# ywyue/AGILE3D

Measured on AMD Instinct MI355X. Metric: scenes/s (80k-voxel, 10 clicks), higher is better.
Workload: dtype f32; 1 GPU; batch of 16 synthetic 79736-voxel scenes, 10 clicks each (5 objects x 2), scene build + forward_backbone + 1 forward_mask per scene, fp32, eval; voxels=79736, queries=20, parallelism=scene-sharded x1 (no data-path collective), global_batch=16, steps_in_flight_per_gpu=4

## Files before the change

### agile3d_amd/csrc/decoder.hip

```cpp
#include "common.h"
#include <algorithm>
#include <type_traits>
#include <vector>

namespace a3d {

typedef float f32x4 __attribute__((ext_vector_type(4)));
#define A3D_GLOBAL __attribute__((address_space(1)))
template <typename T>
__device__ __forceinline__ T gld(const T* p) { return *(const T A3D_GLOBAL*)p; }
template <typename T>
__device__ __forceinline__ void gst(T* p, T v) { *(T A3D_GLOBAL*)p = v; }
__device__ __forceinline__ f32x4 gld4(const float* p) { return *(const f32x4 A3D_GLOBAL*)p; }
__device__ __forceinline__ void gst4(float* p, f32x4 v) { *(f32x4 A3D_GLOBAL*)p = v; }
__device__ __forceinline__ bool block_any(int pred, int* slot) {
  if (threadIdx.x == 0) *slot = 0;
  __syncthreads();
  if (pred) *slot = 1;
  __syncthreads();
  return *(volatile int*)slot != 0;
}
template <typename T>
__device__ __forceinline__ T gld_agent(const T* p) {
  return __hip_atomic_load((const T A3D_GLOBAL*)p, __ATOMIC_RELAXED, __HIP_MEMORY_SCOPE_AGENT);
// ... 17 lines not shown
  return fmaxf(__uint_as_float(b[0]), __uint_as_float(b[1]));
}
__device__ __forceinline__ float rows_sum(float x) {
  auto a = __builtin_amdgcn_permlane16_swap(__float_as_uint(x), __float_as_uint(x), false, false);
  x = __uint_as_float(a[0]) + __uint_as_float(a[1]);
  auto b = __builtin_amdgcn_permlane32_swap(__float_as_uint(x), __float_as_uint(x), false, false);
  return __uint_as_float(b[0]) + __uint_as_float(b[1]);
}
__device__ __forceinline__ float fast_exp(float x) { return __builtin_amdgcn_exp2f(x * 1.4426950408889634f); }
constexpr float kLog2e = 1.4426950408889634f;
constexpr float kPointScoreScale = 0.25f * kLog2e;
__device__ __forceinline__ float exp2_fast(float x) { return __builtin_amdgcn_exp2f(x); }

__device__ __forceinline__ f32x4 mfma4(float a, float b, f32x4 c) { return __builtin_amdgcn_mfma_f32_4x4x1f32(a, b, c, 0, 0, 0); }
__device__ __forceinline__ float rows_sum_scatter(f32x4 s) {
  auto a = __builtin_amdgcn_permlane32_swap(__float_as_uint(s[0]), __float_as_uint(s[1]), false, false);
  auto b = __builtin_amdgcn_permlane32_swap(__float_as_uint(s[2]), __float_as_uint(s[3]), false, false);
  const float r01 = __uint_as_float(a[0]) + __uint_as_float(a[1]);
  const float r23 = __uint_as_float(b[0]) + __uint_as_float(b[1]);
  auto c = __builtin_amdgcn_permlane16_swap(__float_as_uint(r01), __float_as_uint(r23), false, false);
  return __uint_as_float(c[0]) + __uint_as_float(c[1]);
}
__device__ __forceinline__ int row_reg(int g) { return ((g & 1) << 1) | (g >> 1); }
__device__ __forceinline__ float row_bcast(float x, int lane4, int row) {
  return __int_as_float(__builtin_amdgcn_ds_bpermute(lane4 + 64 * row, __float_as_int(x)));
}
__device__ __forceinline__ float quads_max(float x) {
  x = fmaxf(x, __shfl_xor(x, 4, 64));
  return fmaxf(x, __shfl_xor(x, 8, 64));
}
__device__ __forceinline__ float quads_sum(float x) {
  x += __shfl_xor(x, 4, 64);
  return x + __shfl_xor(x, 8, 64);
}

constexpr int kPosBlocks = 16;
struct PosBatch {
  int ns;
  int start[64 + 1];
};
__global__ void __launch_bounds__(256) k_minmax_partial_b(const float* __restrict__ xyz, const PosBatch pb, float* part) {
  __shared__ float s[6][256];
  const int b = blockIdx.y, r0 = pb.start[b], r1 = pb.start[b + 1];
  float mn[3] = {3.4e38f, 3.4e38f, 3.4e38f}, mx[3] = {-3.4e38f, -3.4e38f, -3.4e38f};
  for (int i = r0 + blockIdx.x * 256 + threadIdx.x; i < r1; i += gridDim.x * 256) {
#pragma unroll
    for (int a = 0; a < 3; ++a) {
      const float v = xyz[3 * (size_t)i + a];
      mn[a] = fminf(mn[a], v);
      mx[a] = fmaxf(mx[a], v);
    }
  }
#pragma unroll
  for (int a = 0; a < 3; ++a) {
    s[a][threadIdx.x] = mn[a];
    s[3 + a][threadIdx.x] = mx[a];
  }
  __syncthreads();
  for (int o = 128; o > 0; o >>= 1) {
    if (threadIdx.x < o) {
#pragma unroll
      for (int a = 0; a < 3; ++a) {
        s[a][threadIdx.x] = fminf(s[a][threadIdx.x], s[a][threadIdx.x + o]);
        s[3 + a][threadIdx.x] = fmaxf(s[3 + a][threadIdx.x], s[3 + a][threadIdx.x + o]);
      }
    }
    __syncthreads();
  }
  if (threadIdx.x < 6) part[((size_t)b * gridDim.x + blockIdx.x) * 6 + threadIdx.x] = s[threadIdx.x][0];
}
__global__ void k_minmax_final(const float* __restrict__ part, int nb, float* minmax) {
  part += (size_t)blockIdx.x * nb * 6;
  minmax += 6 * blockIdx.x;
  const int a = threadIdx.x >> 6, lane = threadIdx.x & 63;
  float v = a < 3 ? 3.4e38f : -3.4e38f;
  for (int b = lane; b < nb; b += 64) v = a < 3 ? fminf(v, part[b * 6 + a]) : fmaxf(v, part[b * 6 + a]);
#pragma unroll
  for (int o = 32; o > 0; o >>= 1) {
    const float w = __shfl_xor(v, o, 64);
    v = a < 3 ? fminf(v, w) : fmaxf(v, w);
  }
  if (lane == 0) minmax[a] = v;
}
template <bool NORM>
__device__ __forceinline__ void fourier_row(const float* __restrict__ xyz, size_t i, int jj, const float* __restrict__ gaussB,
                                            const float* __restrict__ minmax, float* out) {
  const float two_pi = 6.283185307179586f;
  float p = 0.f;
#pragma unroll
  for (int a = 0; a < 3; ++a) {
    float u = xyz[3 * i + a];
    if (NORM) {
      const float mn = minmax[a], mx = minmax[3 + a];
      u = (u - mn) / (mx - mn);
    }
    u *= two_pi;
    p += u * gaussB[a * 64 + jj];
  }
  float sn, cs;
  sincosf(p, &sn, &cs);
  out[i * D + jj] = sn;
  out[i * D + 64 + jj] = cs;
}
template <bool NORM>
__global__ void k_fourier_b(const float* __restrict__ xyz, const PosBatch pb, const float* __restrict__ gaussB,
                            const float* __restrict__ minmax, float* out) {
  const int b = blockIdx.y, r0 = pb.start[b], r1 = pb.start[b + 1];
  const size_t e = (size_t)blockIdx.x * blockDim.x + threadIdx.x;
  const size_t i = (size_t)r0 + (e >> 6);
  if (i >= (size_t)r1) return;
  fourier_row<NORM>(xyz, i, (int)(e & 63), gaussB, minmax + 6 * b, out);
}

__device__ const float kSineDimT[64] = {
    1.0f, 1.519911f, 2.3101296f, 3.5111918f, 5.3366995f, 8.111309f, 12.328468f, 18.738173f,
    28.480362f, 43.287613f, 65.79333f, 100.0f, 151.99113f, 231.01291f, 351.11914f, 533.6699f,
    811.131f, 1232.8464f, 1873.8174f, 2848.0361f, 4328.762f, 6579.331f, 1.0f, 1.5505158f,
    2.4040992f, 3.727594f, 5.779693f, 8.961505f, 13.894957f, 21.54435f, 33.404854f, 51.79475f,
    80.30857f, 124.51974f, 193.06982f, 299.3578f, 464.15897f, 719.6858f, 1115.8842f, 1730.1959f,
    2682.696f, 4159.5625f, 6449.467f, 1.0f, 1.5505158f, 2.4040992f, 3.727594f, 5.779693f,
    8.961505f, 13.894957f, 21.54435f, 33.404854f, 51.79475f, 80.30857f, 124.51974f, 193.06982f,
    299.3578f, 464.15897f, 719.6858f, 1115.8842f, 1730.1959f, 2682.696f, 4159.5625f, 6449.467f};
template <bool NORM>
__device__ __forceinline__ void sine_quad(const float* __restrict__ xyz, size_t i, int c4, const float* __restrict__ minmax,
                                          float* out) {
  const float two_pi = 6.283185307179586f;
  float4 v;
  float* vp = &v.x;
#pragma unroll
  for (int h = 0; h < 2; ++h) {
    const int p = 2 * c4 + h;
    const int a = (p >= 22) + (p >= 43);
    float u = xyz[3 * i + a];
    if (NORM) {
      const float mn = minmax[a], mx = minmax[3 + a];
      u = (u - mn) / (mx - mn);
    }
    u *= two_pi;
    sincosf(u / kSineDimT[p], &vp[2 * h], &vp[2 * h + 1]);
  }
  *reinterpret_cast<float4*>(out + i * D + 4 * c4) = v;
}
template <bool NORM>
__global__ void k_sine_b(const float* __restrict__ xyz, const PosBatch pb, const float* __restrict__ minmax, float* out) {
  const int b = blockIdx.y, r0 = pb.start[b], r1 = pb.start[b + 1];
  const size_t e = (size_t)blockIdx.x * blockDim.x + threadIdx.x;
  const size_t i = (size_t)r0 + (e >> 5);
  if (i >= (size_t)r1) return;
  sine_quad<NORM>(xyz, i, (int)(e & 31), minmax + 6 * b, out);
}

constexpr int kLegRows = 32, kLegF = 22, kLegLd = 6 * kLegF;
__device__ __forceinline__ void legacy_rows(const float* __restrict__ xyz, size_t r0, int rows, const float* __restrict__ inv_freq,
                                            float* out, float (*s)[kLegLd]) {
  for (int t = threadIdx.x; t < rows * 3 * kLegF; t += blockDim.x) {
    const int r = t / (3 * kLegF), q = t - 3 * kLegF * r, a = q / kLegF, j = q - kLegF * a;
    float sn, cs;
    sincosf(xyz[3 * (r0 + r) + a] * inv_freq[j], &sn, &cs);
    s[r][2 * kLegF * a + j] = sn;
    s[r][2 * kLegF * a + kLegF + j] = cs;
  }
  __syncthreads();
  for (int t = threadIdx.x; t < rows * 32; t += blockDim.x) {
    const int r = t >> 5, c4 = t & 31;
    *reinterpret_cast<float4*>(out + (r0 + r) * D + 4 * c4) = *reinterpret_cast<const float4*>(&s[r][4 * c4]);
  }
}
__global__ void __launch_bounds__(256) k_legacy_b(const float* __restrict__ xyz, const PosBatch pb,
                                                  const float* __restrict__ inv_freq, float* out) {
  __shared__ __align__(16) float s[kLegRows][kLegLd];
  const int b = blockIdx.y, r1 = pb.start[b + 1];
  const size_t r0 = (size_t)pb.start[b] + (size_t)blockIdx.x * kLegRows;
  if (r0 >= (size_t)r1) return;
  legacy_rows(xyz, r0, (int)((size_t)r1 - r0 < (size_t)kLegRows ? (size_t)r1 - r0 : (size_t)kLegRows), inv_freq, out, s);
}

struct QueryMeta {
  int n_fg, n_bg_click, n_bgl, nq, K;
  int row[A3D_MAX_QUERIES];
  int time[A3D_MAX_QUERIES];
  int obj[A3D_MAX_QUERIES];
  int qrange[A3D_MAX_QUERIES + 2];
};

struct QueryBufs {
  float *queries, *qpos, *qproj, *ks, *vs, *E;
  float *attn, *tmp, *tgt, *qk, *vc, *hidden;
  unsigned* sync;
};
constexpr int kQlMaxHelpers = 8;
constexpr int kMaxQBlocks = A3D_MAX_QUERIES / 32;

struct QuerySample {
  const QueryMeta* meta;
// ... 1989 lines not shown
        for (int t = 0; t < 4; ++t) facc[qt][t] += gld_agent(part + (size_t)(qt * 16 + 4 * g + t) * D + 16 * wave + j);
    }
  }
  qstore_b<QT>(facc, vec_l[V_FFN_B2 + cw], 1.f, false, xa, kQLD, 16 * wave, QP);
  __syncthreads();
  qln16<QT>(cur, xa, Q, vec_l + V_FFN_NW, vec_l + V_FFN_NB, cur, deleg ? nullptr : xa, qpos, B.queries, deleg ? B.tgt : nullptr);
  if (deleg) {
    __builtin_amdgcn_s_waitcnt(0x0F70);
    __syncthreads();
    if (tid == 0) gst_agent(flags + 8, 1u);
  } else {
    __syncthreads();
  }
  qln16<QT>(cur, nullptr, Q, vec_l + V_DN_W, vec_l + V_DN_B, xb, nullptr, nullptr, nullptr, nullptr);
  if (!deleg) {
    qzero<QT>(acc);
    qmm<QT>(xa, wfd, acc);
    qstore_b<QT, true>(acc, vec_l[V_S2C_IN_B + D + cw], kPointScoreScale, false, B.ks, D, 16 * wave, Q);
    qload_p(W.mpack + kMpW0, 8, wave, 0, wfd);
    qzero<QT>(acc);
    qmm<QT>(cur, wfa, acc);
    qstore_b<QT, true>(acc, vec_l[V_S2C_IN_B + 2 * D + cw], 1.f, false, B.vs, D, 16 * wave, Q);
    qload_p(W.mpack + kMpW2, 8, wave, 0, wfa);
    if (W.next_c2s_in_wt) {
      qload_p(W.next_qpack + kQpC2sQ, 8, wave, 0, wfb);
      qzero<QT>(acc);
      qmm<QT>(xa, wfb, acc);
      qstore_b<QT, true>(acc, vec_l[V_NEXT_B + cw], kPointScoreScale, false, B.qproj, D, 16 * wave, Q);
    }
  }
  __syncthreads();
  qzero<QT>(acc);
  qmm<QT>(xb, wfd, acc);
  qstore_b<QT>(acc, vec_l[V_M_B0 + cw], 1.f, true, qpos, kQLD, 16 * wave, QP);
  __syncthreads();
  qzero<QT>(acc);
  qmm<QT>(qpos, wfa, acc);
  qstore_b<QT, true>(acc, vec_l[V_M_B2 + cw], 1.f, false, B.E, D, 16 * wave, Q);
}

}

using namespace a3d;

static int posenc_run(const char* who, int kind, int normalize, const float* xyz_dev, const int64_t* starts, int n_samples,
                      int part_blocks, const float* table_dev, float* minmax_dev, float* out_dev, void* workspace_dev,
                      size_t workspace_bytes, void* stream) {
  if (kind != A3D_POSENC_FOURIER && kind != A3D_POSENC_SINE && kind != A3D_POSENC_LEGACY) {
    set_error("%s: unknown encoding kind %d", who, kind);
    return A3D_ERR_INVALID;
  }
  const bool mm = normalize && kind != A3D_POSENC_LEGACY;
  if ((kind != A3D_POSENC_SINE && !table_dev) || (mm && !minmax_dev) || !out_dev) {
    set_error("%s: bad arguments (table_dev: gauss_B / inv_freq; minmax_dev where the encoding normalises)", who);
    return A3D_ERR_INVALID;
  }
  if (!xyz_dev || !starts || n_samples < 1 || n_samples > 64) {
    set_error("%s: bad arguments (1..64 samples)", who);
    return A3D_ERR_INVALID;
  }
  PosBatch pb;
  pb.ns = n_samples;
  int n_max = 0;
  for (int b = 0; b <= n_samples; ++b) {
    if (starts[b] < 0 || starts[b] > ((int64_t)1 << 30) || (b && starts[b] <= starts[b - 1])) {
      set_error("%s: sample %d has no rows (1..2^30 rows in all, starts must ascend)", who, b - 1);
      return A3D_ERR_INVALID;
    }
    pb.start[b] = (int)starts[b];
    if (b) n_max = std::max(n_max, pb.start[b] - pb.start[b - 1]);
  }
  const size_t part_bytes = (size_t)n_samples * part_blocks * 6 * 4;
  if (mm && (!workspace_dev || workspace_bytes < part_bytes)) {
    set_error("%s: workspace needs >= %zu bytes", who, part_bytes);
    return A3D_ERR_WORKSPACE;
  }
  hipStream_t st = (hipStream_t)stream;
  ProfScope ps(st, A3D_PROF_POSENC, 0, 0, 3, 128, pb.start[n_samples]);
  if (mm) {
    k_minmax_partial_b<<<dim3(part_blocks, n_samples), 256, 0, st>>>(xyz_dev, pb, (float*)workspace_dev);
    k_minmax_final<<<n_samples, 384, 0, st>>>((const float*)workspace_dev, part_blocks, minmax_dev);
  }
  if (kind == A3D_POSENC_FOURIER) {
    const dim3 g((unsigned)(((size_t)n_max * 64 + 255) / 256), n_samples);
    if (mm) k_fourier_b<true><<<g, 256, 0, st>>>(xyz_dev, pb, table_dev, minmax_dev, out_dev);
    else k_fourier_b<false><<<g, 256, 0, st>>>(xyz_dev, pb, table_dev, nullptr, out_dev);
  } else if (kind == A3D_POSENC_SINE) {
    const dim3 g((unsigned)(((size_t)n_max * 32 + 255) / 256), n_samples);
    if (mm) k_sine_b<true><<<g, 256, 0, st>>>(xyz_dev, pb, minmax_dev, out_dev);
    else k_sine_b<false><<<g, 256, 0, st>>>(xyz_dev, pb, nullptr, out_dev);
  } else {
    k_legacy_b<<<dim3((unsigned)((n_max + kLegRows - 1) / kLegRows), n_samples), 256, 0, st>>>(xyz_dev, pb, table_dev, out_dev);
  }
  A3D_LAUNCH_CHECK();
  return A3D_OK;
}
static int posenc_one(const char* who, int kind, int normalize, const float* xyz_dev, int64_t n, const float* table_dev,
                      float* minmax_dev, float* out_dev, void* workspace_dev, size_t workspace_bytes, void* stream) {
  if (n <= 0 || n > (int64_t)1 << 30) {
    set_error("%s: bad arguments", who);
    return A3D_ERR_INVALID;
  }
  const int64_t starts[2] = {0, n};
  const int nb = (int)((n + 255) / 256 < 256 ? (n + 255) / 256 : 256);
  return posenc_run(who, kind, normalize, xyz_dev, starts, 1, nb, table_dev, minmax_dev, out_dev, workspace_dev,
                    workspace_bytes, stream);
}

extern "C" size_t a3d_posenc_batch_workspace_bytes(int n_samples) {
  return n_samples >= 1 && n_samples <= 64 ? (size_t)n_samples * kPosBlocks * 6 * 4 : 0;
}
static int posenc_aligned(const char* who, const float* out_dev) {
  if (((uintptr_t)out_dev & 15) == 0) return A3D_OK;
  set_error("%s: out_dev must be 16-byte aligned", who);
  return A3D_ERR_INVALID;
}
extern "C" int a3d_posenc(int kind, int normalize, const float* xyz_dev, int64_t n, const float* table_dev, float* minmax_dev,
                          float* out_dev, void* workspace_dev, size_t workspace_bytes, void* stream) {
  if (int rc = posenc_aligned("a3d_posenc", out_dev)) return rc;
  return posenc_one("a3d_posenc", kind, normalize, xyz_dev, n, table_dev, minmax_dev, out_dev, workspace_dev,
                    workspace_bytes, stream);
}
extern "C" int a3d_posenc_batch(int kind, int normalize, const float* xyz_dev, const int64_t* starts_host, int n_samples,
                                const float* table_dev, float* minmax_dev, float* out_dev, void* workspace_dev,
                                size_t workspace_bytes, void* stream) {
  if (int rc = posenc_aligned("a3d_posenc_batch", out_dev)) return rc;
  return posenc_run("a3d_posenc_batch", kind, normalize, xyz_dev, starts_host, n_samples, kPosBlocks, table_dev,
                    minmax_dev, out_dev, workspace_dev, workspace_bytes, stream);
}
extern "C" int a3d_posenc_fourier(const float* xyz_dev, int64_t n, const float* gauss_B_dev, float* minmax_dev,
                                  float* out_dev, void* workspace_dev, size_t workspace_bytes, void* stream) {
  return posenc_one("a3d_posenc_fourier", A3D_POSENC_FOURIER, 1, xyz_dev, n, gauss_B_dev, minmax_dev, out_dev,
                    workspace_dev, workspace_bytes, stream);
}
extern "C" int a3d_posenc_fourier_batch(const float* xyz_dev, const int64_t* starts_host, int n_samples,
                                        const float* gauss_B_dev, float* minmax_dev, float* out_dev, void* workspace_dev,
                                        size_t workspace_bytes, void* stream) {
  return posenc_run("a3d_posenc_fourier_batch", A3D_POSENC_FOURIER, 1, xyz_dev, starts_host, n_samples, kPosBlocks,
                    gauss_B_dev, minmax_dev, out_dev, workspace_dev, workspace_bytes, stream);
}

static int check_weights(const a3d_decoder_weights* w) {
  if (!w || w->n_layers < 1 || w->n_layers > A3D_MAX_DEC_LAYERS || w->n_bg_queries < 0 ||
      w->n_bg_queries > A3D_MAX_QUERIES || w->dim_ff % 128 != 0) {
    set_error("decoder: bad weight struct");
    return A3D_ERR_INVALID;
  }
  return A3D_OK;
}

static int check_packs(const a3d_decoder_weights* w) {
  if (!w->mask_pack) {
    set_error("a3d_decoder_forward: the decoder weights carry no mask-head pack (a3d_decoder_pack_query_weights fills "
              "a3d_decoder_layer::query_pack and a3d_decoder_weights::mask_pack)");
    return A3D_ERR_INVALID;
  }
  for (int l = 0; l < w->n_layers; ++l)
    if (!w->layers[l].query_pack) {
      set_error("a3d_decoder_forward: decoder layer %d carries no query-side pack (a3d_decoder_pack_query_weights fills "
                "a3d_decoder_layer::query_pack and a3d_decoder_weights::mask_pack)", l);
      return A3D_ERR_INVALID;
    }
  return A3D_OK;
}

namespace {
struct DecLayout {
  size_t buf[4], labels, counts, part, meta, desc, q[12], sync, total;
  int qp, nchunk;
// ... 749 lines not shown
```

### agile3d_amd/csrc/spconv.hip

```cpp
#include "common.h"
#include <algorithm>

namespace a3d {

typedef float f32x4 __attribute__((ext_vector_type(4)));

struct ConvArgs {
  const float* in;
  int ldi, n_in;
  const int* nbr;
  int nbr_stride;
  const uint32_t* gmask;
  const float* w;
  int K, cin, cout;
  float* out;
  int ldo, n_out;
  const int* out_map;
  const float* scale;
  const float* shift;
  const float* res;
  int ldr;
  int relu;
  int zero_row;
  int tag_table, tag_level;
// ... 1100 lines not shown
    }
  }
  __syncthreads();
  while (grp < ngroups) {
    f32x4 a[NS];
#pragma unroll
    for (int S = 0; S < NS; ++S) {
      if constexpr (HAS2) a[S] = nx[S] + nx2[S];
      else a[S] = nx[S];
    }
    const int next = grp + stride;
    if (next < ngroups) fetch(next);
    f32x4 acc[NCT];
#pragma unroll
    for (int ct = 0; ct < NCT; ++ct) acc[ct] = (f32x4){0.f, 0.f, 0.f, 0.f};
    {
      static_assert(NCT % 2 == 0, "pairs of 16-column tiles");
      constexpr int NP = NS * NCT / 2;
      const f32x4* Ws = Wl + lane;
      f32x4 c0 = Ws[0], c1 = Ws[64];
#pragma unroll
      for (int pi = 0; pi < NP; ++pi) {
        const int S = pi / (NCT / 2), ct = 2 * (pi % (NCT / 2));
        f32x4 n0 = c0, n1 = c1;
        if (pi + 1 < NP) {
          n0 = Ws[(2 * pi + 2) * 64];
          n1 = Ws[(2 * pi + 3) * 64];
        }
        __builtin_amdgcn_sched_barrier(0);
#pragma unroll
        for (int t = 0; t < 4; ++t) {
          acc[ct] = __builtin_amdgcn_mfma_f32_16x16x4f32(c0[t], a[S][t], acc[ct], 0, 0, 0);
          acc[ct + 1] = __builtin_amdgcn_mfma_f32_16x16x4f32(c1[t], a[S][t], acc[ct + 1], 0, 0, 0);
        }
        __builtin_amdgcn_sched_barrier(0);
        c0 = n0;
        c1 = n1;
      }
    }
    if (grp * 16 + j < n) {
      const int row = out_map ? out_map[grp * 16 + j] : grp * 16 + j;
#pragma unroll
      for (int ct = 0; ct < NCT; ++ct) {
        const int col = 16 * ct + 4 * g;
        f32x4 v = acc[ct];
        if (scale) v *= *(const f32x4*)(scale + col);
        if (shift) v += *(const f32x4*)(shift + col);
        if (res) v += *(const f32x4*)(res + (size_t)row * ldr + col);
        if (relu) {
#pragma unroll
          for (int t = 0; t < 4; ++t) v[t] = fmaxf(v[t], 0.f);
        }
        *(f32x4*)(Y + (size_t)row * ldy + col) = v;
      }
    }
    grp = next;
  }
}

static bool dense_supported(int cin, int cout) {
  return (cin == 96 || cin == 128) && (cout == 96 || cout == 128);
}
static int launch_dense(const float* X, int ldx, const float* X2, int ldx2, int n, int cin, int cout, const float* Wp,
                        const float* scale, const float* shift, const float* res, int ldr, int relu, float* Y,
                        int ldy, int zero_row, int tag_level, const int* out_map, hipStream_t st) {
  if ((ldx | ldx2 | ldr | ldy) & 3) {
    set_error("a3d_linear: leading dimensions must be multiples of 4");
    return A3D_ERR_INVALID;
  }
  const int ngroups = (n + 15) / 16;
  const int nw = n >= 200000 ? 12 : 4, wg_per_cu = n >= 200000 ? 1 : 2;
  const size_t lds = (size_t)(cin / 16) * (cout / 16) * 1024;
  ProfScope ps(st, A3D_PROF_DENSE, 0, 1, cin, cout, n, A3D_OP_LINEAR, tag_level, 1);
  const int max_grid = 256 * wg_per_cu;
  const int grid = (ngroups + nw - 1) / nw < max_grid ? (ngroups + nw - 1) / nw : max_grid;
#define A3D_DENSE(NS_, NCT_) (X2 ? big_lds<k_dense<NS_, NCT_, true>>() : big_lds<k_dense<NS_, NCT_, false>>())
  const auto kern = cin == 128 ? (cout == 128 ? A3D_DENSE(8, 8) : A3D_DENSE(8, 6)) : (cout == 128 ? A3D_DENSE(6, 8) : A3D_DENSE(6, 6));
#undef A3D_DENSE
  kern<<<grid, 64 * nw, lds, st>>>(X, ldx, X2, ldx2, n, Wp, scale, shift, res, ldr, relu, Y, ldy, ngroups, zero_row, out_map);
  A3D_LAUNCH_CHECK();
  return A3D_OK;
}

template <int NT, int KS>
__global__ void __launch_bounds__(NT) k_stem(const int32_t* __restrict__ xyzb, int n,
                                              const uint64_t* __restrict__ hk, const int* __restrict__ hv,
                                              uint32_t hmask, const f32x4* __restrict__ feats4,
                                              const float* __restrict__ w, int ,
                                              const float* __restrict__ scale, const float* __restrict__ shift,
                                              int relu, float* out, int ldo, int zero_row, const Level glv) {
  extern __shared__ __attribute__((aligned(16))) char smem[];
  constexpr int ks = KS, K = KS * KS * KS;
  float* W = (float*)smem;
  int* nb = (int*)(W + K * 96);
  const int tid = threadIdx.x;
  for (int e = tid; e < K * 96; e += NT) W[e] = w[e];
  const int v0 = blockIdx.x * 64;
  const int h = ks / 2;
  constexpr int TPV = NT / 64, CPT = 32 / TPV;
  constexpr int SEG = (K + TPV - 1) / TPV;
  const int v = tid / TPV, cg = tid % TPV;
  const bool fused = glv.grid && n < (1 << 25);
  const int mrow = v0 + v;
  const int row = fused ? (mrow < n ? glv.perm[mrow] : n) : mrow;
  int mine[SEG];
  if (fused) {
    int4 c = (int4){0, 0, 0, 0};
    if (mrow < n) {
      int b_, X_, Y_, Z_;
      decode_key(glv.keys[mrow], 0, b_, X_, Y_, Z_);
      c = (int4){X_, Y_, Z_, b_};
    }
#pragma unroll
    for (int u = 0; u < SEG; ++u) {
      const int k = cg * SEG + u;
      mine[u] = -1;
      if (k < K && row < n)
        mine[u] = glv.grid[grid_cell(glv, c.w, c.x + (k % ks) - h, c.y + ((k / ks) % ks) - h, c.z + (k / (ks * ks)) - h)];
    }
  } else if (glv.grid) {
    for (int e0 = tid; e0 < 64 * K; e0 += 8 * NT) {
      int res[8];
#pragma unroll
      for (int u = 0; u < 8; ++u) {
        const int e = e0 + u * NT;
        const int vv = e / K, k = e - vv * K;
        const int rr = v0 + vv;
        res[u] = -1;
        if (e < 64 * K && rr < n) {
          const int4 c = *(const int4*)(xyzb + 4 * rr);
          res[u] = glv.grid[grid_cell(glv, c.w, c.x + (k % ks) - h, c.y + ((k / ks) % ks) - h, c.z + (k / (ks * ks)) - h)];
          if (res[u] >= 0) res[u] = glv.perm[res[u]];
        }
      }
#pragma unroll
      for (int u = 0; u < 8; ++u)
        if (e0 + u * NT < 64 * K) nb[e0 + u * NT] = res[u];
    }
  } else
  for (int e0 = tid; e0 < 64 * K; e0 += 4 * NT) {
    uint64_t key[4];
    uint32_t hh[4];
    int res[4];
    bool open[4];
#pragma unroll
    for (int u = 0; u < 4; ++u) {
      const int e = e0 + u * NT;
      const int v = e / K, k = e - v * K;
      const int row = v0 + v;
      res[u] = -1;
      open[u] = false;
      key[u] = 0;
      hh[u] = 0;
      if (e < 64 * K && row < n) {
        const int X = xyzb[4 * row + 0] + (k % ks) - h;
        const int Y = xyzb[4 * row + 1] + ((k / ks) % ks) - h;
        const int Z = xyzb[4 * row + 2] + (k / (ks * ks)) - h;
        const int b = xyzb[4 * row + 3];
        const int lim = kCoordOff;
        if (X >= -lim && X < lim && Y >= -lim && Y < lim && Z >= -lim && Z < lim) {
          key[u] = make_key(b, X, Y, Z, 0);
          hh[u] = hash64(key[u]) & hmask;
          open[u] = true;
        }
      }
    }
    for (uint32_t probe = 0; probe <= hmask; ++probe) {
      uint64_t got[4];
#pragma unroll
      for (int u = 0; u < 4; ++u) got[u] = open[u] ? hk[hh[u]] : kEmptyKey;
      bool any = false;
#pragma unroll
      for (int u = 0; u < 4; ++u) {
        if (!open[u]) continue;
        if (got[u] == key[u]) {
          res[u] = hv[hh[u]];
          open[u] = false;
        } else if (got[u] == kEmptyKey) {
          open[u] = false;
        } else {
          hh[u] = (hh[u] + 1) & hmask;
          any = true;
        }
      }
      if (!any) break;
    }
#pragma unroll
    for (int u = 0; u < 4; ++u)
      if (e0 + u * NT < 64 * K) nb[e0 + u * NT] = res[u];
  }
  __syncthreads();
  float acc[CPT];
#pragma unroll
  for (int c = 0; c < CPT; ++c) acc[c] = 0.f;
  if (n < (1 << 25)) {
    constexpr int seg = SEG;
    int cnt = 0;
#pragma unroll
    for (int u = 0; u < SEG; ++u) {
      const int k = cg * seg + u;
      if (!fused) mine[u] = k < K ? nb[v * K + k] : -1;
      cnt += mine[u] >= 0 ? 1 : 0;
    }
    int incl = cnt;
#pragma unroll
    for (int o = 1; o < TPV; o <<= 1) {
      const int t = __shfl_up(incl, o, 64);
      if (cg >= o) incl += t;
    }
    const int total = __shfl(incl, (threadIdx.x & 63) | (TPV - 1), 64);
    if (!fused) __syncthreads();
    int pos = incl - cnt;
#pragma unroll
    for (int u = 0; u < SEG; ++u)
      if (mine[u] >= 0) nb[v * K + pos++] = (int)((uint32_t)mine[u] | ((uint32_t)(cg * seg + u) << 25));
    __syncthreads();
    for (int i0 = 0; i0 < total; i0 += 8) {
      uint32_t e[8];
      f32x4 f[8];
#pragma unroll
      for (int u = 0; u < 8; ++u) e[u] = i0 + u < total ? (uint32_t)nb[v * K + i0 + u] : 0u;
#pragma unroll
      for (int u = 0; u < 8; ++u) f[u] = feats4[e[u] & 0x1ffffffu];
#pragma unroll
      for (int u = 0; u < 8; ++u) {
        if (i0 + u >= total) continue;
        const float* wk = W + (e[u] >> 25) * 96 + cg * CPT;
#pragma unroll
        for (int c = 0; c < CPT; ++c) acc[c] += f[u][0] * wk[c] + f[u][1] * wk[32 + c] + f[u][2] * wk[64 + c];
      }
    }
  } else
  for (int k0 = 0; k0 < K; k0 += 5) {
    int r[5];
    f32x4 f[5];
#pragma unroll
    for (int u = 0; u < 5; ++u) r[u] = k0 + u < K ? nb[v * K + k0 + u] : -1;
#pragma unroll
    for (int u = 0; u < 5; ++u) f[u] = feats4[r[u] >= 0 ? r[u] : 0];
#pragma unroll
    for (int u = 0; u < 5; ++u) {
      if (r[u] < 0) continue;
      const float* wk = W + (k0 + u) * 96 + cg * CPT;
#pragma unroll
      for (int c = 0; c < CPT; ++c) acc[c] += f[u][0] * wk[c] + f[u][1] * wk[32 + c] + f[u][2] * wk[64 + c];
    }
  }
  if (row < n) {
#pragma unroll
    for (int c = 0; c < CPT; ++c) {
      const int col = cg * CPT + c;
      float y = acc[c] * (scale ? scale[col] : 1.f) + (shift ? shift[col] : 0.f);
      if (relu) y = fmaxf(y, 0.f);
      out[(size_t)row * ldo + col] = y;
    }
  }
  if (zero_row >= 0 && blockIdx.x == 0 && tid < 32) out[(size_t)zero_row * ldo + tid] = 0.f;
}

__global__ void k_gather_feats(const float* __restrict__ feats3, const int* __restrict__ orig_row, int n,
                               f32x4* feats4, const int* __restrict__ perm) {
  const int f = blockIdx.x * blockDim.x + threadIdx.x;
  if (f >= n) return;
  const float* p = feats3 + (size_t)orig_row[perm ? perm[f] : f] * 3;
  feats4[f] = (f32x4){p[0], p[1], p[2], 0.f};
}

__global__ void k_pack_weight(const float* __restrict__ w, int K, int cin, int cout, float* out) {
  const size_t e = (size_t)blockIdx.x * blockDim.x + threadIdx.x;
  const size_t total = (size_t)K * cin * cout;
  if (e >= total) return;
  const int t = (int)(e & 3), lane = (int)((e >> 2) & 63);
  size_t rest = e >> 8;
  const int cout16 = cout >> 4, cin16 = cin >> 4;
  const int ct = (int)(rest % cout16);
  rest /= cout16;
  const int S = (int)(rest % cin16);
  const int k = (int)(rest / cin16);
  const int g = lane >> 4, j = lane & 15;
  out[e] = w[((size_t)k * cin + 16 * S + 4 * g + t) * cout + 16 * ct + j];
}

constexpr int kMaxQueuesPerOp = 1024;
constexpr int kSkMaxG = 1020;

enum ConvFamily { kConvWl, kConvDeep, kConvSk };
struct ConvPlan {
  ConvFamily family;
  int bn, ch, pair;
  int D, P;
  int G, n_cblk, ntile, nchunk, nchunk2, ov;
  bool handoff, prio;
  bool fused_ok, head_ok;
  size_t lds, slab_floats;
};

static int sk_ch(int cin, int bn) {
  if (cin % 32) return 0;
  if (bn == 128 || bn == 96) return 32;
  const int cand[3] = {96, 64, 32};
  for (int i = 0; i < 3; ++i)
    if (cin % cand[i] == 0 && 2 * cand[i] * bn * 4 + 64 <= 80 * 1024) return cand[i];
  return 0;
}
static int sk_pair(int bn, int ch, int n_rows) {
  if (bn == 128) return ch == 32 && n_rows >= 8192;
  return bn == 96;
}
static int sk_wgs_per_cu(int bn, int ch, int pair, size_t lds) {
  int by_regs = 2;
  if (pair) {
    by_regs = (bn <= 96 && ch <= 32) ? 4 : 3;
  } else {
    if (bn == 32) by_regs = ch <= 32 ? 5 : 4;
    else if (bn == 64) by_regs = ch <= 32 ? 4 : 3;
  }
  const int by_lds = (int)(160 * 1024 / lds);
  const int w = by_regs < by_lds ? by_regs : by_lds;
  return w < 1 ? 1 : (w > 4 ? 4 : w);
}
static ConvPlan plan_sk(int n_rows, int K, int cin, int cout, bool handoff, int force_ch = 0) {
  ConvPlan p;
  memset(&p, 0, sizeof(p));
  p.family = kConvSk;
  p.handoff = handoff;
  p.ntile = (n_rows + 63) / 64;
  if (p.ntile < 1) p.ntile = 1;
  const int k_eff = K == 27 ? 13 : K;
  int gmax = 512;
  for (int pass = 0; pass < 2; ++pass) {
    p.bn = (cout % 128 == 0) ? 128 : cout;
    if (pass == 1 && cout % 64 == 0 && p.bn > 64) p.bn = 64;
    p.ch = force_ch > 0 && cin % force_ch == 0 ? force_ch : sk_ch(cin, p.bn);
    p.nchunk = p.ch ? cin / p.ch : 1;
    p.n_cblk = cout / p.bn;
    p.pair = sk_pair(p.bn, p.ch, n_rows);
    const int mfma_per_stage = p.ch / 4 * (p.bn / 16);
    p.ov = mfma_per_stage >= 128 ? 1 : mfma_per_stage >= 64 ? 2 : 3;
// ... 456 lines not shown
  ProgLayout L;
  if (i < 0 || i >= n_bufs || layout_program(s, bufs, n_bufs, nullptr, 0, L) != A3D_OK) return (size_t)-1;
  return L.buf_off[i];
}

extern "C" int a3d_program_run(const a3d_scene* s, const a3d_buf_desc* bufs, int n_bufs, const a3d_op* ops,
                               int n_ops, const float* feats3_dev, float* ext_out_dev, int ext_out_ld,
                               void* workspace_dev, size_t workspace_bytes, void* stream) {
  ProgLayout L;
  int rc = layout_program(s, bufs, n_bufs, ops, n_ops, L);
  if (rc != A3D_OK) return rc;
  if (!workspace_dev || workspace_bytes < L.total || ((uintptr_t)workspace_dev & 255)) {
    set_error("a3d_program_run: workspace too small or misaligned (%zu < %zu)", workspace_bytes, L.total);
    return A3D_ERR_WORKSPACE;
  }
  hipStream_t st = (hipStream_t)stream;
  char* ws = (char*)workspace_dev;
  f32x4* feats4 = (f32x4*)(ws + L.feats4_off);
  float* partial = (float*)(ws + L.partial_off);
  int* queues = (int*)(ws + L.queue_off);
  A3D_HIP_CHECK(hipMemsetAsync(queues, 0, (size_t)n_ops * kMaxQueuesPerOp * 4, st));
  bool feats_ready = false;
  auto slice = [&](int id, int coff, int ch, int level, int* ld) -> float* {
    if (id < 0 || id >= n_bufs || bufs[id].level != level || coff + ch > bufs[id].channels) return nullptr;
    *ld = bufs[id].channels;
    return (float*)(ws + L.buf_off[id]) + coff;
  };

  for (int i = 0; i < n_ops; ++i) {
    const a3d_op& o = ops[i];
    const int Lin = o.level_in;
    if (Lin < 0 || Lin >= A3D_NUM_LEVELS) {
      set_error("op %d: bad level", i);
      return A3D_ERR_INVALID;
    }
    float* out = nullptr;
    int ldo = 0;
    const int* out_map = nullptr;
    int zero_row = -1;
    const int lvl_out = level_out(o.kind, Lin);
    if (o.out_buf == A3D_BUF_EXT_OUT) {
      if (!ext_out_dev || lvl_out != 0 || o.kind == A3D_OP_UP) {
        set_error("op %d: external output needs a level-0, non-transposed op", i);
        return A3D_ERR_INVALID;
      }
      out = ext_out_dev + o.out_coff;
      ldo = ext_out_ld;
      out_map = s->orig_row;
    } else {
      out = slice(o.out_buf, o.out_coff, o.cout, lvl_out, &ldo);
      if (!out) {
        set_error("op %d: bad output buffer", i);
        return A3D_ERR_INVALID;
      }
      zero_row = s->lv[lvl_out].n;
    }
    const float* res = nullptr;
    int ldr = 0;
    if (o.res_buf != A3D_BUF_NONE) {
      res = slice(o.res_buf, o.res_coff, o.cout, lvl_out, &ldr);
      if (!res || o.out_buf == A3D_BUF_EXT_OUT) {
        set_error("op %d: bad residual buffer", i);
        return A3D_ERR_INVALID;
      }
    }

    if (o.kind == A3D_OP_STEM) {
      if (Lin != 0 || o.cin != 3 || o.cout != 32 || !feats3_dev ||
          !(o.kernel_volume == 125 || o.kernel_volume == 27)) {
        set_error("op %d: stem expects level 0, 3->32 channels, 5^3 or 3^3 kernel", i);
        return A3D_ERR_UNSUPPORTED;
      }
      const Level& lv = s->lv[0];
      const int ks = o.kernel_volume == 125 ? 5 : 3;
      const bool morton = lv.grid && ks / 2 <= kGridPad && lv.n < (1 << 25);
      if (!feats_ready) {
        k_gather_feats<<<(lv.n + 255) / 256, 256, 0, st>>>(feats3_dev, s->orig_row, lv.n, feats4, morton ? lv.perm : nullptr);
        feats_ready = true;
      }
      const size_t lds = (size_t)o.kernel_volume * 96 * 4 + (size_t)64 * o.kernel_volume * 4;
      ProfScope ps(st, A3D_PROF_STEM, 0, o.kernel_volume, 3, 32, lv.n);
      Level glv = lv;
      if (ks / 2 > kGridPad) glv.grid = nullptr;
      (ks == 5 ? k_stem<512, 5> : k_stem<512, 3>)<<<(lv.n + 63) / 64, 512, lds, st>>>(
          lv.xyzb, lv.n, lv.hkeys, lv.hvals, lv.hmask, feats4, o.w_dev, ks, o.scale_dev, o.shift_dev, o.relu, out, ldo, zero_row, glv);
      A3D_LAUNCH_CHECK();
      continue;
    }

    ConvArgs a;
    memset(&a, 0, sizeof(a));
    a.in = slice(o.in_buf, o.in_coff, o.cin, Lin, &a.ldi);
    if (!a.in) {
      set_error("op %d: bad input buffer", i);
      return A3D_ERR_INVALID;
    }
    a.n_in = s->lv[Lin].n, a.w = o.w_dev, a.K = o.kernel_volume, a.cin = o.cin, a.cout = o.cout;
    a.out = out, a.ldo = ldo, a.out_map = out_map, a.n_out = s->lv[lvl_out].n, a.zero_row = zero_row;
    a.scale = o.scale_dev, a.shift = o.shift_dev, a.res = res, a.ldr = ldr, a.relu = o.relu;
    a.tag_table = o.kind, a.tag_level = Lin;
    if (o.proj_cin > 0) {
      a.in2 = slice(o.proj_buf, o.proj_coff, o.proj_cin, Lin, &a.ldi2);
      if (o.kind != A3D_OP_CONV3 || !a.in2 || o.scale_dev) {
        set_error("op %d: bad fused projection", i);
        return A3D_ERR_INVALID;
      }
      a.cin2 = o.proj_cin;
    }
    const int* pre = nullptr;
    if (!bind_tables(s, o.kind, Lin, a, &pre)) {
      set_error("op %d: unknown kind %d", i, o.kind);
      return A3D_ERR_INVALID;
    }
    if (o.kernel_volume != kind_volume(o.kind)) {
      static const char* const what[] = {"CONV3 needs kernel volume 27", "bad DOWN", "bad UP", "LINEAR needs kernel volume 1"};
      set_error("op %d: %s", i, what[o.kind - A3D_OP_CONV3]);
      return A3D_ERR_INVALID;
    }
    ConvPlan plan = {};
    if (o.head_cout > 0 || a.cin2 > 0) {
      ConvShape shape = conv_shape(a, 0, true, L.partial_floats);
      shape.head_cout = o.head_cout;
      plan = plan_conv(shape);
    }
    bool head_after = false;
    if (o.head_cout > 0) {
      if (!o.head_w_dev || !ext_out_dev || lvl_out != 0 || o.kind == A3D_OP_UP || o.out_buf == A3D_BUF_EXT_OUT ||
          o.head_cout % 16 || o.head_cout > ext_out_ld) {
        set_error("op %d: a fused head needs a level-0 op into a buffer, packed head weights and the external output", i);
        return A3D_ERR_INVALID;
      }
      if (o.kind != A3D_OP_LINEAR && plan.head_ok) {
        a.head_w = o.head_w_dev;
        a.head_bias = o.head_bias_dev;
        a.head_out = ext_out_dev;
        a.head_ld = ext_out_ld;
        a.head_cout = o.head_cout;
        a.head_map = s->orig_row;
      } else {
        head_after = true;
      }
    }
    if (a.cin2 > 0 && !plan.fused_ok) {
      ConvArgs c1 = a;
      c1.in2 = nullptr, c1.cin2 = 0, c1.ldi2 = 0, c1.relu = 0;
      rc = launch_conv_sk(c1, pre, partial, L.partial_floats, queues + (size_t)i * kMaxQueuesPerOp, st);
      if (rc != A3D_OK) return rc;
      if (a.out_map) {
        set_error("op %d: fused projection has no fallback for a row-mapped output", i);
        return A3D_ERR_UNSUPPORTED;
      }
      ConvArgs c2 = linear_args(a.in2, a.ldi2, a.n_out, a.cin2, a.cout, a.w + (size_t)27 * a.cin * a.cout, a.out, a.ldo, Lin);
      c2.res = a.out, c2.ldr = a.ldo, c2.relu = a.relu, c2.zero_row = a.zero_row;
      rc = launch_conv_sk(c2, nullptr, nullptr, 0, nullptr, st);
      if (rc != A3D_OK) return rc;
    } else
    if (o.kind == A3D_OP_LINEAR && dense_supported(a.cin, a.cout) && a.n_out >= 4096)
      rc = launch_dense(a.in, a.ldi, nullptr, 0, a.n_out, a.cin, a.cout, a.w, a.scale, a.shift, a.res, a.ldr, a.relu,
                        a.out, a.ldo, a.zero_row, Lin, a.out_map, st);
    else
      rc = launch_conv_sk(a, pre, partial, L.partial_floats, queues + (size_t)i * kMaxQueuesPerOp, st);
    if (rc != A3D_OK) return rc;
    if (head_after) {
      if (dense_supported(o.cout, o.head_cout) && a.n_out >= 4096)
        rc = launch_dense(out, ldo, nullptr, 0, a.n_out, o.cout, o.head_cout, o.head_w_dev, nullptr, o.head_bias_dev, nullptr, 0, 0,
                          ext_out_dev, ext_out_ld, -1, Lin, s->orig_row, st);
      else {
// ... 164 lines not shown
```

Before: 649.5 scenes/s.

## Vectorize normalized Fourier posenc and make stem kernel persistent with prefetched lookups

Adds a Fourier positional-encoding kernel for the normalized path where each thread computes four frequencies, uses float4 loads and stores when aligned, and uses hardware sin/cos on range-reduced turns in place of sincosf. The stem convolution becomes a persistent grid capped at 512 blocks that loops over tiles and prefetches the next tile's key and neighbor lookups while the current tile computes, with grid lookups taken from a precomputed corner offset. The stem also pins FMA rounding through a helper and adds a waves-per-EU hint. The fast sin/cos and the changed rounding may shift numerics, and the persistent loop cuts the number of blocks launched.

```diff
diff --git a/agile3d_amd/csrc/decoder.hip b/agile3d_amd/csrc/decoder.hip
--- a/agile3d_amd/csrc/decoder.hip
+++ b/agile3d_amd/csrc/decoder.hip
@@ -123,34 +123,64 @@
   }
   if (lane == 0) minmax[a] = v;
 }
-template <bool NORM>
-__device__ __forceinline__ void fourier_row(const float* __restrict__ xyz, size_t i, int jj, const float* __restrict__ gaussB,
-                                            const float* __restrict__ minmax, float* out) {
+__global__ void k_fourier_b(const float* __restrict__ xyz, const PosBatch pb, const float* __restrict__ gaussB, float* out) {
+  const int b = blockIdx.y, r0 = pb.start[b], r1 = pb.start[b + 1];
+  const size_t e = (size_t)blockIdx.x * blockDim.x + threadIdx.x;
+  const size_t i = (size_t)r0 + (e >> 6);
+  if (i >= (size_t)r1) return;
+  const int jj = (int)(e & 63);
   const float two_pi = 6.283185307179586f;
   float p = 0.f;
 #pragma unroll
-  for (int a = 0; a < 3; ++a) {
-    float u = xyz[3 * i + a];
-    if (NORM) {
-      const float mn = minmax[a], mx = minmax[3 + a];
-      u = (u - mn) / (mx - mn);
-    }
-    u *= two_pi;
-    p += u * gaussB[a * 64 + jj];
-  }
+  for (int a = 0; a < 3; ++a) p += xyz[3 * i + a] * two_pi * gaussB[a * 64 + jj];
   float sn, cs;
   sincosf(p, &sn, &cs);
   out[i * D + jj] = sn;
   out[i * D + 64 + jj] = cs;
 }
-template <bool NORM>
-__global__ void k_fourier_b(const float* __restrict__ xyz, const PosBatch pb, const float* __restrict__ gaussB,
-                            const float* __restrict__ minmax, float* out) {
+template <bool A16>
+__global__ void __launch_bounds__(256) k_fourier_rev(const float* __restrict__ xyz, const PosBatch pb,
+                                                     const float* __restrict__ gaussB, const float* __restrict__ minmax,
+                                                     float* out) {
   const int b = blockIdx.y, r0 = pb.start[b], r1 = pb.start[b + 1];
   const size_t e = (size_t)blockIdx.x * blockDim.x + threadIdx.x;
-  const size_t i = (size_t)r0 + (e >> 6);
+  const size_t i = (size_t)r0 + (e >> 4);
   if (i >= (size_t)r1) return;
-  fourier_row<NORM>(xyz, i, (int)(e & 63), gaussB, minmax + 6 * b, out);
+  const int j0 = 4 * (int)(e & 15);
+  minmax += 6 * b;
+  float t[4] = {0.f, 0.f, 0.f, 0.f};
+#pragma unroll
+  for (int a = 0; a < 3; ++a) {
+    const float mn = minmax[a], mx = minmax[3 + a];
+    const float u = (xyz[3 * i + a] - mn) / (mx - mn);
+    float w[4];
+    if (A16) {
+      *reinterpret_cast<float4*>(w) = *reinterpret_cast<const float4*>(gaussB + a * 64 + j0);
+    } else {
+#pragma unroll
+      for (int k = 0; k < 4; ++k) w[k] = gaussB[a * 64 + j0 + k];
+    }
+#pragma unroll
+    for (int k = 0; k < 4; ++k) t[k] += u * w[k];
+  }
+  float sn[4], cs[4];
+#pragma unroll
+  for (int k = 0; k < 4; ++k) {
+    const float r = t[k] - rintf(t[k]);
+    sn[k] = __builtin_amdgcn_sinf(r);
+    cs[k] = __builtin_amdgcn_cosf(r);
+  }
+  float* o = out + i * D + j0;
+  if (A16) {
+    *reinterpret_cast<float4*>(o) = *reinterpret_cast<const float4*>(sn);
+    *reinterpret_cast<float4*>(o + 64) = *reinterpret_cast<const float4*>(cs);
+  } else {
+#pragma unroll
+    for (int k = 0; k < 4; ++k) {
+      o[k] = sn[k];
+      o[64 + k] = cs[k];
+    }
+  }
 }
 
 __device__ const float kSineDimT[64] = {
@@ -2306,9 +2336,14 @@
     k_minmax_final<<<n_samples, 384, 0, st>>>((const float*)workspace_dev, part_blocks, minmax_dev);
   }
   if (kind == A3D_POSENC_FOURIER) {
-    const dim3 g((unsigned)(((size_t)n_max * 64 + 255) / 256), n_samples);
-    if (mm) k_fourier_b<true><<<g, 256, 0, st>>>(xyz_dev, pb, table_dev, minmax_dev, out_dev);
-    else k_fourier_b<false><<<g, 256, 0, st>>>(xyz_dev, pb, table_dev, nullptr, out_dev);
+    if (mm) {
+      const dim3 g((unsigned)(((size_t)n_max * 16 + 255) / 256), n_samples);
+      if ((((uintptr_t)out_dev | (uintptr_t)table_dev) & 15) == 0)
+        k_fourier_rev<true><<<g, 256, 0, st>>>(xyz_dev, pb, table_dev, minmax_dev, out_dev);
+      else k_fourier_rev<false><<<g, 256, 0, st>>>(xyz_dev, pb, table_dev, minmax_dev, out_dev);
+    } else {
+      k_fourier_b<<<dim3((unsigned)(((size_t)n_max * 64 + 255) / 256), n_samples), 256, 0, st>>>(xyz_dev, pb, table_dev, out_dev);
+    }
   } else if (kind == A3D_POSENC_SINE) {
     const dim3 g((unsigned)(((size_t)n_max * 32 + 255) / 256), n_samples);
     if (mm) k_sine_b<true><<<g, 256, 0, st>>>(xyz_dev, pb, minmax_dev, out_dev);
diff --git a/agile3d_amd/csrc/spconv.hip b/agile3d_amd/csrc/spconv.hip
--- a/agile3d_amd/csrc/spconv.hip
+++ b/agile3d_amd/csrc/spconv.hip
@@ -1206,8 +1206,18 @@
   return A3D_OK;
 }
 
+template <int CPT>
+__device__ __forceinline__ void stem_accumulate(float (&acc)[CPT], const f32x4& f, const float* __restrict__ wk) {
+#pragma clang fp contract(off)
+  static_assert(CPT == 4, "the pinned roundings are those of the four-channel build");
+#pragma unroll
+  for (int c = 0; c < CPT; ++c) {
+    const float t = __builtin_fmaf(f[0], wk[c], f[1] * wk[32 + c]);
+    acc[c] += c < CPT / 2 ? __builtin_fmaf(f[2], wk[64 + c], t) : t + f[2] * wk[64 + c];
+  }
+}
 template <int NT, int KS>
-__global__ void __launch_bounds__(NT) k_stem(const int32_t* __restrict__ xyzb, int n,
+__global__ void __launch_bounds__(NT) __attribute__((amdgpu_waves_per_eu(4))) k_stem(const int32_t* __restrict__ xyzb, int n,
                                               const uint64_t* __restrict__ hk, const int* __restrict__ hv,
                                               uint32_t hmask, const f32x4* __restrict__ feats4,
                                               const float* __restrict__ w, int ,
@@ -1219,29 +1229,46 @@
   int* nb = (int*)(W + K * 96);
   const int tid = threadIdx.x;
   for (int e = tid; e < K * 96; e += NT) W[e] = w[e];
-  const int v0 = blockIdx.x * 64;
   const int h = ks / 2;
   constexpr int TPV = NT / 64, CPT = 32 / TPV;
   constexpr int SEG = (K + TPV - 1) / TPV;
   const int v = tid / TPV, cg = tid % TPV;
   const bool fused = glv.grid && n < (1 << 25);
-  const int mrow = v0 + v;
-  const int row = fused ? (mrow < n ? glv.perm[mrow] : n) : mrow;
+  const int ntiles = (n + 63) >> 6;
   int mine[SEG];
-  if (fused) {
-    int4 c = (int4){0, 0, 0, 0};
-    if (mrow < n) {
-      int b_, X_, Y_, Z_;
-      decode_key(glv.keys[mrow], 0, b_, X_, Y_, Z_);
-      c = (int4){X_, Y_, Z_, b_};
-    }
+  uint64_t key_nx = 0;
+  int row_nx = n;
+  auto fetch_key = [&](int tile) {
+    const int mr = tile * 64 + v;
+    row_nx = n;
+    if (tile < ntiles && mr < n) {
+      key_nx = glv.keys[mr];
+      row_nx = glv.perm[mr];
+    }
+  };
+  auto lookups = [&]() {
+    int b_, X_, Y_, Z_;
+    decode_key(key_nx, 0, b_, X_, Y_, Z_);
+    const int* corner = glv.grid + grid_cell(glv, b_, X_ - h, Y_ - h, Z_ - h);
 #pragma unroll
     for (int u = 0; u < SEG; ++u) {
       const int k = cg * SEG + u;
       mine[u] = -1;
-      if (k < K && row < n)
-        mine[u] = glv.grid[grid_cell(glv, c.w, c.x + (k % ks) - h, c.y + ((k / ks) % ks) - h, c.z + (k / (ks * ks)) - h)];
-    }
+      if (k < K && row_nx < n) mine[u] = corner[((k / (ks * ks)) * glv.gdim[1] + (k / ks) % ks) * glv.gdim[0] + k % ks];
+    }
+  };
+  int row_f = n;
+  if (fused) {
+    fetch_key(blockIdx.x);
+    lookups();
+    row_f = row_nx;
+  }
+  for (int tile = blockIdx.x; tile < ntiles; tile += gridDim.x) {
+  const int v0 = tile * 64;
+  const int mrow = v0 + v;
+  const int row = fused ? row_f : mrow;
+  if (fused) {
+    fetch_key(tile + gridDim.x);
   } else if (glv.grid) {
     for (int e0 = tid; e0 < 64 * K; e0 += 8 * NT) {
       int res[8];
@@ -1338,6 +1365,10 @@
 #pragma unroll
     for (int u = 0; u < SEG; ++u)
       if (mine[u] >= 0) nb[v * K + pos++] = (int)((uint32_t)mine[u] | ((uint32_t)(cg * seg + u) << 25));
+    if (fused) {
+      lookups();
+      row_f = row_nx;
+    }
     __syncthreads();
     for (int i0 = 0; i0 < total; i0 += 8) {
       uint32_t e[8];
@@ -1349,9 +1380,7 @@
 #pragma unroll
       for (int u = 0; u < 8; ++u) {
         if (i0 + u >= total) continue;
-        const float* wk = W + (e[u] >> 25) * 96 + cg * CPT;
-#pragma unroll
-        for (int c = 0; c < CPT; ++c) acc[c] += f[u][0] * wk[c] + f[u][1] * wk[32 + c] + f[u][2] * wk[64 + c];
+        stem_accumulate<CPT>(acc, f[u], W + (e[u] >> 25) * 96 + cg * CPT);
       }
     }
   } else
@@ -1365,9 +1394,7 @@
 #pragma unroll
     for (int u = 0; u < 5; ++u) {
       if (r[u] < 0) continue;
-      const float* wk = W + (k0 + u) * 96 + cg * CPT;
-#pragma unroll
-      for (int c = 0; c < CPT; ++c) acc[c] += f[u][0] * wk[c] + f[u][1] * wk[32 + c] + f[u][2] * wk[64 + c];
+      stem_accumulate<CPT>(acc, f[u], W + (k0 + u) * 96 + cg * CPT);
     }
   }
   if (row < n) {
@@ -1378,6 +1405,8 @@
       if (relu) y = fmaxf(y, 0.f);
       out[(size_t)row * ldo + col] = y;
     }
+  }
+  if (!fused) __syncthreads();
   }
   if (zero_row >= 0 && blockIdx.x == 0 && tid < 32) out[(size_t)zero_row * ldo + tid] = 0.f;
 }
@@ -2000,7 +2029,8 @@
       ProfScope ps(st, A3D_PROF_STEM, 0, o.kernel_volume, 3, 32, lv.n);
       Level glv = lv;
       if (ks / 2 > kGridPad) glv.grid = nullptr;
-      (ks == 5 ? k_stem<512, 5> : k_stem<512, 3>)<<<(lv.n + 63) / 64, 512, lds, st>>>(
+      const int tiles = (lv.n + 63) / 64;
+      (ks == 5 ? k_stem<512, 5> : k_stem<512, 3>)<<<tiles < 512 ? tiles : 512, 512, lds, st>>>(
           lv.xyzb, lv.n, lv.hkeys, lv.hvals, lv.hmask, feats4, o.w_dev, ks, o.scale_dev, o.shift_dev, o.relu, out, ldo, zero_row, glv);
       A3D_LAUNCH_CHECK();
       continue;
```

Measured after the change: 649.3 scenes/s. About the same (-0.0%).
